# SRainGit/CAE-LO

Hardware: AMD Instinct MI355X
Metric: KITTI frames/sec end-to-end (keypts+desc+match+RANSAC) (higher is better)
Workload: dtype f32

## Files before the change

cae-lo_amd/csrc/encoder.hip:

```cpp
#include <math.h>

#include "caelo_internal.h"
#include <vector>
#include <stdlib.h>
#include <string.h>

typedef float f32x4 __attribute__((ext_vector_type(4)));

#define MFMA16(a, b, c) __builtin_amdgcn_mfma_f32_16x16x4f32((a), (b), (c), 0, 0, 0)

__device__ inline float enc_tanh(float x) {
    const float e = __builtin_amdgcn_exp2f(x * 2.8853900817779268f);
    return 1.0f - 2.0f * __builtin_amdgcn_rcpf(e + 1.0f);
}

#define DENSE_N 200
#define DENSE_NP 208
#define DENSE_K 2048
#define C3X_NPAIR 14
#define C3X_TICKET_INT 512
static void conv3_split_weights(const float *w3, uint4 *out);
static void stage1x_split_weights(const float *w1, const float *w2, uint4 *w1f, uint4 *w2x);
int enc_upload_dense1(const float *wd1, const float *bd1, int K, void **wx_dev, float **bd_dev);
#define HEAD_WQ_FLOATS (13 * 2 * 64 * 4)
// ... 247 lines not shown
                    const unsigned int n2 = (((w1 & 0xFFFFu) << 1) >> sh) & 0xFu, n3 = (((w1 >> 16) << 1) >> sh) & 0xFu;
                    m32[a >> 1] |= (n0 | (n1 << 4) | (n2 << 8) | (n3 << 12)) << ((a & 1) * 16);
                }
                cmask[rep] = (unsigned long long)m32[0] | ((unsigned long long)m32[1] << 32);
            }
        }
        int j_fetch;
        if (tid == 0) j_fetch = atomicAdd(work_counter, 1);
        ENC_STAMP(1);
#pragma unroll
        for (int rep = 0; rep < 2; ++rep) {
            const int cell = tid + rep * 256;
            const bool hit = cmask[rep] != 0ull;
            const unsigned long long bal = __ballot(hit);
            if (bal != 0ull) {
                int base = 0;
                if (lane == 0) base = atomicAdd(&L.list_n, __popcll(bal));
                base = __shfl(base, 0);
                if (hit) {
                    L.list_cell[base + __popcll(bal & ((1ull << lane) - 1ull))] = (unsigned short)cell;
                    L.cell_mask[cell] = cmask[rep];
                    atomicOr(&L.nzrow[(cell >> 6) + 1], 1u << (((cell >> 3) & 7) + 1));
                }
            }
        }
        caelo_lds_barrier();
        ENC_STAMP(2);
        const int nlist = L.list_n;
        for (int base = wave * 8; base < nlist; base += 32) {
            const int item = base + (lane >> 3);
            const int sub = lane & 7;
            float acc[8];
            int cell = 0;
            if (item < nlist) {
                cell = L.list_cell[item];
                const unsigned long long mask = L.cell_mask[cell];
                const int sa = sub >> 2, sb = (sub >> 1) & 1, sc = sub & 1;
                unsigned int taps = 0;
#pragma unroll
                for (int ka = 0; ka < 3; ++ka)
#pragma unroll
                    for (int kb = 0; kb < 3; ++kb)
                        taps |= ((unsigned int)(mask >> ((sa + ka) * 16 + (sb + kb) * 4 + sc)) & 7u) << ((ka * 3 + kb) * 3);
#pragma unroll
                for (int c = 0; c < 8; ++c) acc[c] = L.b1[c];
                while (taps) {
                    const int t = __ffs((int)taps) - 1;
                    taps &= taps - 1;
                    const float4 wa = *(const float4 *)&L.w1[t * 8], wb = *(const float4 *)&L.w1[t * 8 + 4];
                    acc[0] += wa.x; acc[1] += wa.y; acc[2] += wa.z; acc[3] += wa.w;
                    acc[4] += wb.x; acc[5] += wb.y; acc[6] += wb.z; acc[7] += wb.w;
                }
            } else {
#pragma unroll
                for (int c = 0; c < 8; ++c) acc[c] = -3.0e38f;
            }
#pragma unroll
            for (int c = 0; c < 8; ++c) {
                acc[c] = fmaxf(acc[c], __int_as_float(__builtin_amdgcn_update_dpp(0, __float_as_int(acc[c]), 0xB1, 0xF, 0xF, true)));
                acc[c] = fmaxf(acc[c], __int_as_float(__builtin_amdgcn_update_dpp(0, __float_as_int(acc[c]), 0x4E, 0xF, 0xF, true)));
                acc[c] = fmaxf(acc[c], __int_as_float(__builtin_amdgcn_update_dpp(0, __float_as_int(acc[c]), 0x141, 0xF, 0xF, true)));
            }
            if (item < nlist) {
                float mine = acc[0];
#pragma unroll
                for (int c = 1; c < 8; ++c) mine = (sub == c) ? acc[c] : mine;
                const int px = cell >> 6, py = (cell >> 3) & 7, pz = cell & 7;
                const int q = ((px + 1) * 10 + (py + 1)) * 10 + pz + 1;
                L.p1[(sub >> 2) * S1P_PLANE + q * 4 + (sub & 3)] = enc_tanh(mine) - L.bg[sub];
            }
        }
        if (tid == 0) L.next_j = (int)gridDim.x + j_fetch;
        caelo_lds_barrier();
        ENC_STAMP(3);
        const int jn = __builtin_amdgcn_readfirstlane(L.next_j);
        unsigned int row_next = 0u;
        if (jn < n_items) {
            const unsigned long long *src;
            enc_item(in, jn, nk, group, src, patch_next);
            patch_next = __builtin_amdgcn_readfirstlane(patch_next);
            row_next = ((const unsigned short *)src)[tid];
        }
        {
            const int yl = n >> 3, z = n & 7;
            const float *plane = L.p1 + (g >> 1) * S1P_PLANE + 2 * (g & 1);
#pragma unroll
            for (int yi = 0; yi < 4; ++yi) {
                const int y0 = 2 * yi;
                const int xp = wave ^ S1_XDEAL(yi);
                const unsigned int r0 = (unsigned)__builtin_amdgcn_readfirstlane((int)((L.nzrow[2 * xp] >> y0) & 0xFu));
                const unsigned int r1 = (unsigned)__builtin_amdgcn_readfirstlane((int)((L.nzrow[2 * xp + 1] >> y0) & 0xFu));
                const unsigned int r2 = (unsigned)__builtin_amdgcn_readfirstlane((int)((L.nzrow[2 * xp + 2] >> y0) & 0xFu));
                const unsigned int r3 = (unsigned)__builtin_amdgcn_readfirstlane((int)((L.nzrow[2 * xp + 3] >> y0) & 0xFu));
                float *dst = p2out + (size_t)patch * 1024 + (size_t)(((xp * 4 + yi) * 4 + 2 * (g & 1)) * 16 + n);
                if ((r0 | r1 | r2 | r3) == 0u) {
                    if (g < 2) {
                        const float2 o = L.bgout[wave][yi][lane];
                        dst[0] = o.x; dst[16] = o.y;
                    }
                    continue;
                }
                f32x4 acc0 = c0r[yi][0];
                f32x4 acc1 = c0r[yi][1];
                f32x4 acc0b = {0.f, 0.f, 0.f, 0.f}, acc1b = {0.f, 0.f, 0.f, 0.f};
                const int qbase = ((2 * xp) * 10 + (y0 + yl)) * 10 + z + 1;
                const float *a0 = plane + qbase * 4;
                const float *a1 = a0 + 100 * 4;
                CONV2Z_TILE(acc0, acc0b, a0, r0, r1, r2)
                CONV2Z_TILE(acc1, acc1b, a1, r1, r2, r3)
                acc0 += acc0b;
                acc1 += acc1b;
                float v0 = fmaxf(fmaxf(acc0[0], acc0[1]), fmaxf(acc1[0], acc1[1]));
                float v1 = fmaxf(fmaxf(acc0[2], acc0[3]), fmaxf(acc1[2], acc1[3]));
                v0 = fmaxf(v0, __shfl_xor(v0, 32));
                v1 = fmaxf(v1, __shfl_xor(v1, 32));
                if (g < 2) {
                    dst[0] = enc_tanh(v0);
                    dst[16] = enc_tanh(v1);
                }
            }
        }
        caelo_lds_barrier();
        ENC_STAMP(4);
#ifdef CAELO_ENC_PROF
        if (threadIdx.x == 0) { L.prof[6] += 1; L.prof[7] += nlist; }
#else
        if (threadIdx.x == 0 && blockIdx.x == 0 && patch == 0) g_enc_stamp[8] = (unsigned long long)nlist;
#endif
        for (int i = tid; i < nlist * 2; i += 256) {
            const int cell = L.list_cell[i >> 1];
            const int px = cell >> 6, py = (cell >> 3) & 7, pz = cell & 7;
            const int q = ((px + 1) * 10 + (py + 1)) * 10 + pz + 1;
            *(float4 *)&L.p1[(i & 1) * S1P_PLANE + q * 4] = make_float4(0.f, 0.f, 0.f, 0.f);
        }
        if (tid == 0) L.list_n = 0;
        if (tid < 12) L.nzrow[tid] = 0u;
        L.rows[rbuf ^ 1][row_slot] = (unsigned short)row_next;
        rbuf ^= 1;
        caelo_lds_barrier();
        j = jn;
        row = row_next;
        patch = patch_next;
        ENC_STAMP(5);
    }
#ifdef CAELO_ENC_PROF
    if (threadIdx.x == 0)
        for (int i = 0; i < 8; ++i) atomicAdd(&g_enc_stamp[i], (unsigned long long)L.prof[i]);
#endif
}

#include "enc_stage1x.inc"

#define ENC_XCD_CSTRIDE 32
#define C3X_PLANE 48
#define C3X_ARR 292
#define C3X_SPLIT (2 * C3X_ARR)
#ifndef C3X_F16
#define C3X_F16 1
#endif
#define C3X_NS (C3X_F16 ? 2 : 3)
#define C3X_SLOT (C3X_NS * C3X_SPLIT)
typedef __bf16 bf16x8 __attribute__((ext_vector_type(8)));
__host__ __device__ constexpr int c3x_pairA(int p) { return p < 9 ? p * 3 : (p < 12 ? (p - 9) * 9 + 2 : (p == 12 ? 8 : 26)); }
__host__ __device__ constexpr int c3x_pairB(int p) { return p < 9 ? p * 3 + 1 : (p < 12 ? (p - 9) * 9 + 5 : (p == 12 ? 17 : -1)); }
__host__ __device__ constexpr int c3x_pairClass(int p) { return p < 9 ? 0 : (p < 12 ? 1 : (p == 12 ? 2 : 3)); }
__host__ __device__ constexpr int c3x_tapPos(int t) { return (t / 9) * C3X_PLANE + ((t / 3) % 3) * 8 + (t % 3); }
__host__ __device__ constexpr bool c3x_dead(int x, int p) {
    return (x == 0 && c3x_pairA(p) / 9 == 0 && (c3x_pairB(p) < 0 || c3x_pairB(p) / 9 == 0)) ||
           (x == 3 && c3x_pairA(p) / 9 == 2 && (c3x_pairB(p) < 0 || c3x_pairB(p) / 9 == 2));
}

__host__ __device__ inline uint32_t enc_bf16_rne(float x) {
    union { float f; uint32_t u; } v = {x};
    return (v.u + 0x7FFFu + ((v.u >> 16) & 1u)) & 0xFFFF0000u;
}
__host__ __device__ inline float enc_bits_f32(uint32_t u) {
    union { uint32_t u; float f; } v = {u};
    return v.f;
}
__host__ __device__ inline void enc_split3(float x, uint32_t &hi, uint32_t &mid, uint32_t &lo) {
    hi = enc_bf16_rne(x);
    const float r = x - enc_bits_f32(hi);
    mid = enc_bf16_rne(r);
    lo = enc_bf16_rne(r - enc_bits_f32(mid));
}
__device__ inline void enc_split3_pk(float x0, float x1, uint32_t &hi, uint32_t &mid, uint32_t &lo) {
    typedef __bf16 enc_bf2 __attribute__((ext_vector_type(2)));
    typedef float enc_f2 __attribute__((ext_vector_type(2)));
    hi = __builtin_bit_cast(uint32_t, __builtin_convertvector((enc_f2){x0, x1}, enc_bf2));
    const float r0 = x0 - __uint_as_float(hi << 16), r1 = x1 - __uint_as_float(hi & 0xFFFF0000u);
    mid = __builtin_bit_cast(uint32_t, __builtin_convertvector((enc_f2){r0, r1}, enc_bf2));
    const float q0 = r0 - __uint_as_float(mid << 16), q1 = r1 - __uint_as_float(mid & 0xFFFF0000u);
    lo = __builtin_bit_cast(uint32_t, __builtin_convertvector((enc_f2){q0, q1}, enc_bf2));
}
__device__ inline void enc_split2h_pk(float x0, float x1, uint32_t &hi, uint32_t &lo) {
    const _Float16 h0 = (_Float16)x0, h1 = (_Float16)x1;
    const _Float16 l0 = (_Float16)(x0 - (float)h0), l1 = (_Float16)(x1 - (float)h1);
    hi = (uint32_t)__builtin_bit_cast(uint16_t, h0) | ((uint32_t)__builtin_bit_cast(uint16_t, h1) << 16);
    lo = (uint32_t)__builtin_bit_cast(uint16_t, l0) | ((uint32_t)__builtin_bit_cast(uint16_t, l1) << 16);
}
#define ENC_PK8(A) make_uint4((A[0] >> 16) | A[1], (A[2] >> 16) | A[3], (A[4] >> 16) | A[5], (A[6] >> 16) | A[7])

static void conv3_split_weights(const float *w3, uint4 *out) {
    for (int nt = 0; nt < 2; ++nt)
        for (int p = 0; p < C3X_NPAIR; ++p)
            for (int lane = 0; lane < 64; ++lane) {
                const int n = lane & 15, g = lane >> 4;
                const int tap = g < 2 ? c3x_pairA(p) : c3x_pairB(p);
                uint4 *o = out + ((size_t)(nt * C3X_NPAIR + p) * C3X_NS) * 64 + lane;
#if C3X_F16
                uint16_t h[8], l[8];
                for (int i = 0; i < 8; ++i)
                    enc_split2h(tap >= 0 ? w3[(tap * 16 + 8 * (g & 1) + i) * 32 + nt * 16 + n] : 0.0f, h[i], l[i]);
                o[0] = make_uint4(h[0] | (uint32_t)h[1] << 16, h[2] | (uint32_t)h[3] << 16, h[4] | (uint32_t)h[5] << 16, h[6] | (uint32_t)h[7] << 16);
                o[64] = make_uint4(l[0] | (uint32_t)l[1] << 16, l[2] | (uint32_t)l[3] << 16, l[4] | (uint32_t)l[5] << 16, l[6] | (uint32_t)l[7] << 16);
#else
                uint32_t h[8], m[8], l[8];
                for (int i = 0; i < 8; ++i)
                    enc_split3(tap >= 0 ? w3[(tap * 16 + 8 * (g & 1) + i) * 32 + nt * 16 + n] : 0.0f, h[i], m[i], l[i]);
                o[0] = ENC_PK8(h);
                o[64] = ENC_PK8(m);
                o[128] = ENC_PK8(l);
#endif
            }
}

#ifndef C3X_WGS
#define C3X_WGS 2
#endif
__global__ void __launch_bounds__(256, C3X_WGS) k_enc_conv3(const float *__restrict__ p2, int64_t n_patches, const caelo_enc_in in,
                                                      const uint4 *__restrict__ w3x, const float *__restrict__ b3g,
                                                      float *__restrict__ f3, int *__restrict__ stage1_counter,
                                                      int *__restrict__ xcd_counters) {
    __shared__ uint4 S[2 * C3X_SLOT];
    if (blockIdx.x == 0 && threadIdx.x == 0) *stage1_counter = 0;
    if (blockIdx.x == 0 && threadIdx.x < 8) xcd_counters[threadIdx.x * ENC_XCD_CSTRIDE] = 0;
    const int tid = threadIdx.x;
    const int lane = tid & 63;
    const int wave = tid >> 6;
    const int g = lane >> 4, n = lane & 15;
    const int ntile = wave & 1, slot = __builtin_amdgcn_readfirstlane(wave >> 1);
    uint4 bq[C3X_NPAIR][C3X_NS];
#pragma unroll
    for (int p = 0; p < C3X_NPAIR; ++p)
#pragma unroll
        for (int sp = 0; sp < C3X_NS; ++sp) bq[p][sp] = w3x[((size_t)(ntile * C3X_NPAIR + p) * C3X_NS + sp) * 64 + lane];
    const float bias = b3g[16 * ntile + n];
    for (int i = tid; i < 2 * C3X_SLOT; i += 256) S[i] = make_uint4(0u, 0u, 0u, 0u);
    __syncthreads();
    const int n_items = enc_items_total(in, n_patches);
    const int n_pairs = (n_items + 1) / 2;
#define C3_ROW(ITEM, ROW)                                     \
    {                                                         \
        ROW = (ITEM);                                         \
        if (in.dedup) {                                       \
            int f_, i_;                                       \
            ROW = enc_item_row(in, (ITEM), f_, i_);           \
        }                                                     \
    }
    const int f_slot = __builtin_amdgcn_readfirstlane(tid >> 7), f_pos = (tid >> 1) & 63, f_h = tid & 1;
    const int f_q = (((f_pos >> 4) + 1) * 6 + ((f_pos >> 2) & 3) + 1) * 8 + (f_pos & 3) + 1;
    float4 pre0, pre1;
#define C3_FETCH(PAIR)                                                                           \
    {                                                                                            \
        const int pa_ = (PAIR) * 2 + f_slot;                                                     \
        pre0 = make_float4(0.f, 0.f, 0.f, 0.f);                                                  \
        pre1 = pre0;                                                                             \
        if ((PAIR) < n_pairs && pa_ < n_items) {                                                 \
            int row_;                                                                            \
            C3_ROW(pa_, row_)                                                                    \
            const float4 *q_ = (const float4 *)(p2 + (size_t)row_ * 1024 + f_pos * 16 + 8 * f_h); \
            pre0 = q_[0];                                                                        \
            pre1 = q_[1];                                                                        \
        }                                                                                        \
    }
#ifdef CAELO_C3_PROF
    unsigned long long c3_t[4] = {0ull, 0ull, 0ull, 0ull};
    unsigned c3_prev = (unsigned)clock64();
#define C3_STAMP(i) do { if (tid == 0) { const unsigned t_ = (unsigned)clock64(); c3_t[i] += t_ - c3_prev; c3_prev = t_; } } while (0)
#else
#define C3_STAMP(i) do { } while (0)
#endif
    __shared__ int s_after[2];
    const int xcd = (int)(blockIdx.x & 7u), wgs_of_xcd = ((int)gridDim.x - xcd + 7) >> 3;
    int *const ticket = stage1_counter + C3X_TICKET_INT + 32 * xcd;
    int pair = xcd + 8 * (int)(blockIdx.x >> 3), next = pair + 8 * wgs_of_xcd;
    int drawn = 0;
    if (tid == 0) drawn = atomicAdd(ticket, 1);
    C3_FETCH(pair)
    for (int it = 0; pair < n_pairs; pair = next, next = __builtin_amdgcn_readfirstlane(s_after[it & 1]), ++it) {
        C3_STAMP(3);
        {
            const float v[8] = {pre0.x, pre0.y, pre0.z, pre0.w, pre1.x, pre1.y, pre1.z, pre1.w};
            uint4 *d = &S[f_slot * C3X_SLOT + f_h * C3X_ARR + f_q];
#if C3X_F16
            uint32_t h[4], l[4];
#pragma unroll
            for (int k = 0; k < 4; ++k) enc_split2h_pk(v[2 * k], v[2 * k + 1], h[k], l[k]);
            d[0] = make_uint4(h[0], h[1], h[2], h[3]);
            d[C3X_SPLIT] = make_uint4(l[0], l[1], l[2], l[3]);
#else
            uint32_t h[4], m[4], l[4];
#pragma unroll
            for (int k = 0; k < 4; ++k) enc_split3_pk(v[2 * k], v[2 * k + 1], h[k], m[k], l[k]);
            d[0] = make_uint4(h[0], h[1], h[2], h[3]);
            d[C3X_SPLIT] = make_uint4(m[0], m[1], m[2], m[3]);
            d[2 * C3X_SPLIT] = make_uint4(l[0], l[1], l[2], l[3]);
#endif
        }
        if (tid == 0) s_after[it & 1] = xcd + 8 * (2 * wgs_of_xcd + drawn);
        C3_STAMP(0);
        __syncthreads();
        C3_STAMP(1);
        if (tid == 0) drawn = atomicAdd(ticket, 1);
        C3_FETCH(next)
        const int item = pair * 2 + slot;
        int patch;
        C3_ROW(item, patch)
        const uint4 *base = &S[slot * C3X_SLOT + (g & 1) * C3X_ARR + (n >> 2) * 8 + (n & 3)];
        const uint4 *ab[4] = {base + (g >= 2 ? 1 : 0), base + (g >= 2 ? 8 : 0), base + (g >= 2 ? C3X_PLANE : 0), base};
#pragma unroll
        for (int round = 0; round < 2; ++round) {
            f32x4 acc[2];
#pragma unroll
            for (int j = 0; j < 2; ++j) acc[j] = (f32x4){bias, bias, bias, bias};
#pragma unroll
            for (int p = 0; p < C3X_NPAIR; ++p) {
#if C3X_F16
                typedef _Float16 c3_h8 __attribute__((ext_vector_type(8)));
                const c3_h8 bh = __builtin_bit_cast(c3_h8, bq[p][0]), bl = __builtin_bit_cast(c3_h8, bq[p][1]);
                c3_h8 ah[2], al[2];
#pragma unroll
                for (int j = 0; j < 2; ++j) {
                    if (c3x_dead(2 * round + j, p)) continue;
                    const uint4 *a = ab[c3x_pairClass(p)] + c3x_tapPos(c3x_pairA(p)) + (2 * round + j) * C3X_PLANE;
                    ah[j] = __builtin_bit_cast(c3_h8, a[0]);
                    al[j] = __builtin_bit_cast(c3_h8, a[C3X_SPLIT]);
                }
#define C3X_MAC(A, B)                                                                                           \
    _Pragma("unroll") for (int j = 0; j < 2; ++j) if (!c3x_dead(2 * round + j, p))                              \
        acc[j] = __builtin_amdgcn_mfma_f32_16x16x32_f16(A[j], B, acc[j], 0, 0, 0);
                C3X_MAC(al, bh)
                C3X_MAC(ah, bl)
                C3X_MAC(ah, bh)
#else
                const bf16x8 bh = __builtin_bit_cast(bf16x8, bq[p][0]), bm = __builtin_bit_cast(bf16x8, bq[p][1]),
                             bl = __builtin_bit_cast(bf16x8, bq[p][2]);
                bf16x8 ah[2], am[2], al[2];
#pragma unroll
                for (int j = 0; j < 2; ++j) {
                    if (c3x_dead(2 * round + j, p)) continue;
                    const uint4 *a = ab[c3x_pairClass(p)] + c3x_tapPos(c3x_pairA(p)) + (2 * round + j) * C3X_PLANE;
                    ah[j] = __builtin_bit_cast(bf16x8, a[0]);
                    am[j] = __builtin_bit_cast(bf16x8, a[C3X_SPLIT]);
                    al[j] = __builtin_bit_cast(bf16x8, a[2 * C3X_SPLIT]);
                }
#define C3X_MAC(A, B)                                                                                           \
    _Pragma("unroll") for (int j = 0; j < 2; ++j) if (!c3x_dead(2 * round + j, p))                              \
        acc[j] = __builtin_amdgcn_mfma_f32_16x16x32_bf16(A[j], B, acc[j], 0, 0, 0);
                C3X_MAC(al, bh)
                C3X_MAC(ah, bl)
                C3X_MAC(am, bm)
                C3X_MAC(am, bh)
                C3X_MAC(ah, bm)
                C3X_MAC(ah, bh)
#endif
            }
            if (item < n_items) {
                float *dst = f3 + (size_t)patch * 2048 + 16 * ntile + n;
#pragma unroll
                for (int j = 0; j < 2; ++j)
#pragma unroll
                    for (int r = 0; r < 4; ++r) dst[(((2 * round + j) * 4 + g) * 4 + r) * 32] = enc_tanh(acc[j][r]);
            }
        }
        C3_STAMP(2);
        __syncthreads();
    }
#ifdef CAELO_C3_PROF
    if (tid == 0) {
        for (int i = 0; i < 4; ++i) atomicAdd(&g_enc_stamp[8 + i], c3_t[i]);
        atomicAdd(&g_enc_stamp[12], 1ull);
    }
#endif
}

#define D1_BM 64
#define D1_BK 32
#define D1_SPLIT 8
#ifndef D1_SPLIT_2048
#define D1_SPLIT_2048 2
#endif
#define D1_SPLIT_OF(KTOT) ((KTOT) > 2048 ? 8 : D1_SPLIT_2048)
#define D1_THREADS 512
#define D1_NT (DENSE_NP / 16)
#define D1_NS 2
#define D1_B16 (D1_NS * D1_NT * 64)
#define D1_BSLOTS ((D1_B16 + D1_THREADS - 1) / D1_THREADS)

static void dense1_split_weights(const float *wd1, int K, uint4 *out) {
    for (int ks = 0; ks < K / 32; ++ks)
        for (int nt = 0; nt < D1_NT; ++nt)
            for (int lane = 0; lane < 64; ++lane) {
                const int n = lane & 15, g = lane >> 4, col = nt * 16 + n;
                uint16_t h[8], l[8];
                for (int i = 0; i < 8; ++i)
                    enc_split2h(col < DENSE_N ? wd1[(size_t)(ks * 32 + 8 * g + i) * DENSE_N + col] : 0.0f, h[i], l[i]);
                uint4 *o = out + (size_t)ks * D1_B16 + nt * 64 + lane;
                o[0] = make_uint4(h[0] | (uint32_t)h[1] << 16, h[2] | (uint32_t)h[3] << 16, h[4] | (uint32_t)h[5] << 16, h[6] | (uint32_t)h[7] << 16);
                o[D1_NT * 64] = make_uint4(l[0] | (uint32_t)l[1] << 16, l[2] | (uint32_t)l[3] << 16, l[4] | (uint32_t)l[5] << 16, l[6] | (uint32_t)l[7] << 16);
            }
}

int enc_upload_dense1(const float *wd1, const float *bd1, int K, void **wx_dev, float **bd_dev) {
    const size_t n = (size_t)(K / 32) * D1_B16;
    uint4 *wx = (uint4 *)malloc(n * sizeof(uint4));
    if (!wx) { caelo_set_error("out of host memory"); return CAELO_ERR_ARG; }
    dense1_split_weights(wd1, K, wx);
    float bd[DENSE_NP] = {0.0f};
    memcpy(bd, bd1, DENSE_N * sizeof(float));
    hipError_t e = hipSuccess;
    if (!*wx_dev) e = hipMalloc(wx_dev, (n + 6 * 64) * sizeof(uint4));
    if (e == hipSuccess && !*bd_dev) e = hipMalloc((void **)bd_dev, sizeof(bd));
    if (e == hipSuccess) e = hipMemcpy(*wx_dev, wx, n * sizeof(uint4), hipMemcpyHostToDevice);
    if (e == hipSuccess) e = hipMemcpy(*bd_dev, bd, sizeof(bd), hipMemcpyHostToDevice);
    free(wx);
    if (e != hipSuccess) { caelo_set_error("dense_1 upload failed: %s", hipGetErrorString(e)); return CAELO_ERR_HIP; }
    return CAELO_OK;
}

typedef _Float16 d1_h8 __attribute__((ext_vector_type(8)));
#define D1_MFMA(A, B, C) __builtin_amdgcn_mfma_f32_16x16x32_f16((A), (B), (C), 0, 0, 0)

#define D1P_BSTRIDE (26 * 64)
#define D1P_NBUF(MTW) 3
#define D1P_LDS_BYTES(MTW) ((2 * D1_NS * 4 * D1_BM * (MTW) + D1P_NBUF(MTW) * D1P_BSTRIDE) * 16)
template <int KTOT, int MTW>
__global__ void __launch_bounds__(D1_THREADS, 2) k_enc_dense1p(const float *__restrict__ f3, int64_t n_rows_pad,
                                                               const uint4 *__restrict__ wd1x, float *__restrict__ part,
                                                               const caelo_enc_in in) {
    constexpr int BM = D1_BM * MTW, A16 = D1_NS * 4 * BM, NBUF = D1P_NBUF(MTW), NKS = KTOT / D1_SPLIT_OF(KTOT) / D1_BK;
    constexpr int DMA = 4;
    constexpr int PER_STAGE = DMA + MTW;
    static_assert(MTW >= 1 && MTW <= 3, "three instances");
    static_assert(NKS % 2 == 0 && NKS >= 6, "stages are unrolled in pairs, the last ones peeled");
    int64_t row0 = (int64_t)blockIdx.x * BM;
    int split = blockIdx.y;
    if (in.dedup) {
        const int lin = (int)(blockIdx.y * gridDim.x + blockIdx.x);
        int t = lin / D1_SPLIT_OF(KTOT), f = 0;
        split = lin - t * D1_SPLIT_OF(KTOT);
        for (; f < in.n_frames; ++f) {
            const int live = (enc_tables(in, f)->count + BM - 1) / BM;
            if (t < live) break;
            t -= live;
        }
        if (f == in.n_frames) return;
        row0 = (int64_t)f * in.per_frame + (int64_t)t * BM;
    }
    extern __shared__ uint4 d1_lds[];
    uint4 *As = d1_lds;
    uint4 *Bs = d1_lds + 2 * A16;
    const int tid = threadIdx.x;
    const int lane = tid & 63, wave = __builtin_amdgcn_readfirstlane(tid >> 6);
    const int g = lane >> 4, n = lane & 15;
    const int ks0 = split * NKS;
    const int mg = wave >> 1;
    const bool odd = (wave & 1) != 0;
    const int nt0 = odd ? 7 : 0;
    f32x4 acc[MTW][7];
#pragma unroll
    for (int q = 0; q < MTW; ++q)
#pragma unroll
        for (int i = 0; i < 7; ++i) acc[q][i] = (f32x4){0.f, 0.f, 0.f, 0.f};
    const int a_row = wave * 8 + ((lane >> 1) & 7), a_kq = ((lane >> 4) << 1) | (lane & 1);
    const float *a_src = f3 + (size_t)(row0 + a_row) * KTOT + (size_t)ks0 * D1_BK + a_kq * 4;
    const int pb = wave < 6 ? 4 * wave : 22;
    const uint32_t b_lds = (uint32_t)(uintptr_t)(void __attribute__((address_space(3))) *)(Bs + (pb + 1) * 64);
    const uint4 *b_mid = wd1x + (size_t)ks0 * D1_B16 + (pb + 1) * 64 + lane;
    const uint32_t a_lds = (uint32_t)(uintptr_t)(void __attribute__((address_space(3))) *)&As[(a_kq >> 1) * BM + a_row] + (a_kq & 1) * 8;
    f32x4 paA[MTW], paB[MTW];
    d1_h8 af0[MTW][D1_NS], af1[MTW][D1_NS], bf0[4][D1_NS], bf1[3][D1_NS];
#define D1P_FETCH_B(KS, BUF)                                                                                     \
    {                                                                                                            \
        const uint4 *gp_ = b_mid + (size_t)(KS) * D1_B16;                                                        \
        const uint32_t la_ = b_lds + (uint32_t)(BUF) * (D1P_BSTRIDE * 16u);                                      \
        __asm__ volatile("s_mov_b32 m0, %0\n\ts_nop 0\n\t"                                                       \
                         "global_load_lds_dwordx4 %1, off offset:-1024\n\t"                                       \
                         "global_load_lds_dwordx4 %1, off\n\tglobal_load_lds_dwordx4 %1, off offset:1024\n\t"    \
                         "global_load_lds_dwordx4 %1, off offset:2048" : : "s"(la_), "v"(gp_) : "memory");       \
    }
#define D1P_LOAD_A(P, KS)                                                                                        \
    _Pragma("unroll") for (int r = 0; r < MTW; ++r) {                                                            \
        const float *p_ = a_src + (size_t)(64 * r) * KTOT + (size_t)(KS) * D1_BK;                                \
        __asm__ volatile("global_load_dwordx4 %0, %1, off" : "=v"(P[r]) : "v"(p_) : "memory");                   \
    }
#define D1P_WAIT_A(P, N)                                                                                         \
    {                                                                                                            \
        if (MTW == 1) __asm__ volatile("s_waitcnt vmcnt(%1)" : "+v"(P[0]) : "n"(N) : "memory");                  \
        else __asm__ volatile("s_waitcnt vmcnt(%2)" : "+v"(P[0]), "+v"(P[MTW - 1]) : "n"(N) : "memory");         \
    }
#define D1P_STORE_A(P, ABUF)                                                                               \
    _Pragma("unroll") for (int r = 0; r < MTW; ++r) {                                                      \
        uint32_t h01_, l01_, h23_, l23_;                                                                   \
        enc_split2h_pk(P[r][0], P[r][1], h01_, l01_);                                                      \
        enc_split2h_pk(P[r][2], P[r][3], h23_, l23_);                                                      \
        const unsigned long long dh_ = ((unsigned long long)h23_ << 32) | h01_, dl_ = ((unsigned long long)l23_ << 32) | l01_; \
        if (r == 0)                                                                                        \
            __asm__ volatile("ds_write_b64 %0, %1 offset:%3\n\tds_write_b64 %0, %2 offset:%4"               \
                             : : "v"(a_lds), "v"(dh_), "v"(dl_), "n"((ABUF) * A16 * 16),                     \
                                 "n"((ABUF) * A16 * 16 + 4 * BM * 16) : "memory");                          \
        else if (r == 1)                                                                                   \
            __asm__ volatile("ds_write_b64 %0, %1 offset:%3\n\tds_write_b64 %0, %2 offset:%4"               \
                             : : "v"(a_lds), "v"(dh_), "v"(dl_), "n"((ABUF) * A16 * 16 + 1024),              \
                                 "n"((ABUF) * A16 * 16 + 4 * BM * 16 + 1024) : "memory");                   \
        else                                                                                               \
            __asm__ volatile("ds_write_b64 %0, %1 offset:%3\n\tds_write_b64 %0, %2 offset:%4"               \
                             : : "v"(a_lds), "v"(dh_), "v"(dl_), "n"((ABUF) * A16 * 16 + 2048),              \
                                 "n"((ABUF) * A16 * 16 + 4 * BM * 16 + 2048) : "memory");                   \
    }
#define D1P_READ_A(AF, ABUF)                                                                               \
    _Pragma("unroll") for (int q = 0; q < MTW; ++q) {                                                      \
        const uint4 *ap_ = &As[(ABUF) * A16 + g * BM + (mg * MTW + q) * 16 + n];                           \
        AF[q][0] = __builtin_bit_cast(d1_h8, ap_[0]);                                                      \
        AF[q][1] = __builtin_bit_cast(d1_h8, ap_[4 * BM]);                                                 \
    }
#define D1P_READ_B0(BUF)                                                                                   \
    {                                                                                                      \
// ... 158 lines not shown
        int r_ = enc_tables(in, (int)f_)->slot_of[p - f_ * per_in];
        if (r_ < 0) {
            const unsigned g_ = (unsigned)(-r_ - 1), fr_ = g_ / per_in;
            r_ = enc_tables(in, (int)fr_)->slot_of[g_ - fr_ * per_in];
        }
        row = (unsigned)r_;
    }
    const float *src = part + (size_t)row * DENSE_NP + 4 * g;
    float4 v[HM_JW][SPLIT];
#pragma unroll
    for (int c = 0; c < HM_JW; ++c)
#pragma unroll
        for (int sp = 0; sp < SPLIT; ++sp)
            if (wave + 4 * c < D1_NT) v[c][sp] = *(const float4 *)(src + (size_t)sp * n_rows_pad * DENSE_NP + 16 * (wave + 4 * c));
    f32x4 acc0 = {0.f, 0.f, 0.f, 0.f}, acc1 = {0.f, 0.f, 0.f, 0.f};
#pragma unroll
    for (int c = 0; c < HM_JW; ++c) {
        if (wave + 4 * c < D1_NT) {
            float4 sum = b1[c];
#pragma unroll
            for (int sp = 0; sp < SPLIT; ++sp) { sum.x += v[c][sp].x; sum.y += v[c][sp].y; sum.z += v[c][sp].z; sum.w += v[c][sp].w; }
            const float hv[4] = {enc_tanh(sum.x), enc_tanh(sum.y), enc_tanh(sum.z), enc_tanh(sum.w)};
            const float w0[4] = {wq[c][0].x, wq[c][0].y, wq[c][0].z, wq[c][0].w}, w1[4] = {wq[c][1].x, wq[c][1].y, wq[c][1].z, wq[c][1].w};
#pragma unroll
            for (int i = 0; i < 4; ++i) {
                acc0 = __builtin_amdgcn_mfma_f32_16x16x4f32(hv[i], w0[i], acc0, 0, 0, 0);
                acc1 = __builtin_amdgcn_mfma_f32_16x16x4f32(hv[i], w1[i], acc1, 0, 0, 0);
            }
        }
    }
    if (wave > 0) {
        s_c[wave - 1][0][lane] = acc0;
        s_c[wave - 1][1][lane] = acc1;
    }
    __syncthreads();
    if (wave > 0) return;
#pragma unroll
    for (int w = 0; w < 3; ++w) {
        acc0 += s_c[w][0][lane];
        acc1 += s_c[w][1][lane];
    }
    const float bo0 = bd2[m], bo1 = m < 4 ? bd2[16 + m] : 0.0f;
#pragma unroll
    for (int i = 0; i < 4; ++i) {
        const unsigned pp = tile * 16u + 4u * (unsigned)g + (unsigned)i;
        if (pp < n_all) {
            const unsigned f = pp / per_out, q = pp - f * per_out, kp = q / (unsigned)group;
            float *dst = outs.base[f] + (size_t)kp * out_stride + (size_t)(q - kp * (unsigned)group) * 20;
            const float d0 = enc_tanh(bo0 + acc0[i]);
            dst[m] = d0;
            if (!(fabsf(d0) <= 1.0f)) atomicAdd(faults, 1);
            if (m < 4) {
                const float d1 = enc_tanh(bo1 + acc1[i]);
                dst[16 + m] = d1;
                if (!(fabsf(d1) <= 1.0f)) atomicAdd(faults, 1);
            }
        }
    }
}

static inline int64_t pad64(int64_t n) { return (n + D1_BM - 1) / D1_BM * D1_BM; }


CAELO_API int64_t caelo_encode_ws_bytes(int64_t n_patches) {
    const int64_t np = pad64(n_patches);
    return CAELO_ENC_WS_HEADER + (np * 1024 + np * 2048 + (int64_t)D1_SPLIT * np * DENSE_NP) * (int64_t)sizeof(float);
}

CAELO_API int caelo_encode_ws_layout(int64_t n_patches, int64_t out[6]) {
    CAELO_REQUIRE(out && n_patches > 0, "caelo_encode_ws_layout: bad argument");
    const int64_t np = pad64(n_patches);
    out[0] = CAELO_ENC_WS_HEADER;
    out[1] = out[0] + np * 1024 * (int64_t)sizeof(float);
    out[2] = out[1] + np * 2048 * (int64_t)sizeof(float);
    out[3] = np;
    out[4] = D1_SPLIT_OF(DENSE_K);
    out[5] = D1_SPLIT;
    return CAELO_OK;
}

int encode_impl(caelo_ctx *c, const uint64_t *bits, int64_t n_patches, int group, float *out, int out_stride,
                       void *ws, hipStream_t s, hipEvent_t *ev ) {
    CAELO_REQUIRE(out, "null argument");
    caelo_enc_out outs;
    outs.base[0] = out;
    outs.per_frame = n_patches > 0 ? n_patches : 1;
    return encode_batch_impl(c, bits, n_patches, group, outs, out_stride, ws, s, ev);
}

int encode_batch_impl(caelo_ctx *c, const uint64_t *bits, int64_t n_patches, int group, const caelo_enc_out &outs,
                      int out_stride, void *ws, hipStream_t s, hipEvent_t *ev , const caelo_enc_in *in) {
    CAELO_REQUIRE(c && bits && ws, "null argument");
    const caelo_enc_in ein = in ? *in : caelo_enc_in{(const unsigned long long *)bits, 0, (int32_t)(n_patches < 0x7FFFFFFF ? n_patches : 0), 1, 0, 0};
    CAELO_REQUIRE(!ein.dedup || (ein.n_frames >= 1 && ein.n_frames <= CAELO_ENC_MAX_FRAMES && ein.per_frame % (3 * D1_BM) == 0 &&
                                 (int64_t)ein.n_frames * ein.per_frame == n_patches),
                  "bad de-duplicated launch");
    CAELO_REQUIRE(outs.per_frame > 0 && (n_patches + outs.per_frame - 1) / outs.per_frame <= CAELO_ENC_MAX_FRAMES, "bad frame table");
    CAELO_REQUIRE(!ein.dedup || ein.per_frame == CAELO_FRAME_PATCHES, "de-duplicated launches hold whole frames of 3072 patches");
    CAELO_REQUIRE(c->has_enc, "encoder weights not set (caelo_set_encoder_weights)");
    CAELO_REQUIRE(n_patches > 0 && n_patches < 0x7FFFFFFF && group >= 1 && out_stride >= group * 20, "bad shape");
    const int64_t np = pad64(n_patches);
    int *work_counter = (int *)ws;
    unsigned long long *mfma_count = (unsigned long long *)((char *)ws + CAELO_ENC_WS_MFMA);
    float *p2 = (float *)((char *)ws + CAELO_ENC_WS_HEADER);
    float *f3 = p2 + np * 1024;
    float *part = f3 + np * 2048;
    if (np > n_patches)
        CAELO_HIP(hipMemsetAsync(f3 + n_patches * 2048, 0, (size_t)(np - n_patches) * 2048 * sizeof(float), s));
    const bool stage1x = !c->enc_reference;
    static int slots1x_slot[CAELO_MAX_DEVICES];
    static bool slots1x_have[CAELO_MAX_DEVICES];
    static std::mutex slots1x_mu;
    const int slots1x = per_device_once(c->device, slots1x_slot, slots1x_have, slots1x_mu, [&] {
        int per_cu = 0, cus = 0;
        if (hipOccupancyMaxActiveBlocksPerMultiprocessor(&per_cu, (const void *)k_enc_stage1x<false>, 256, 0) != hipSuccess ||
            hipDeviceGetAttribute(&cus, hipDeviceAttributeMultiprocessorCount, c->device) != hipSuccess || per_cu * cus <= 0)
            return 512;
        return per_cu * cus;
    });
    int *xcd_counters = (int *)((char *)ws + 1024);
    static int slots1_slot[CAELO_MAX_DEVICES];
    static bool slots1_have[CAELO_MAX_DEVICES];
    static std::mutex slots1_mu;
    const int slots1 = per_device_once(c->device, slots1_slot, slots1_have, slots1_mu, [&] {
        int per_cu = 0, cus = 0;
        if (hipOccupancyMaxActiveBlocksPerMultiprocessor(&per_cu, (const void *)k_enc_stage1, 256, 0) != hipSuccess ||
            hipDeviceGetAttribute(&cus, hipDeviceAttributeMultiprocessorCount, c->device) != hipSuccess || per_cu * cus <= 0)
            return 768;
        return per_cu * cus;
    });
    const int64_t cap1 = (ein.yield & 1) ? (int64_t)slots1 * 4 / 5 : slots1;
    const unsigned g1 = (unsigned)(n_patches < cap1 ? n_patches : cap1);
    if (ev) CAELO_HIP(hipEventRecord(ev[0], s));
    const int order_group = (n_patches % group == 0) ? group : 1;
    if (stage1x) {
        static const int slots_env = getenv("CAELO_S1X_SLOTS") ? atoi(getenv("CAELO_S1X_SLOTS")) : 0;
        const int64_t capx = slots_env > 0 ? slots_env : ((ein.yield & 1) ? (int64_t)slots1x * 2 / 3 : slots1x);
        const unsigned gx = (unsigned)(n_patches < capx ? n_patches : capx);
        if (ev) {
            CAELO_HIP(hipMemsetAsync(mfma_count, 0, 1024, s));
            CAELO_HIP(hipEventRecord(ev[0], s));
            k_enc_stage1x<true><<<gx, 256, 0, s>>>(ein, n_patches, order_group, work_counter, (const uint4 *)c->enc_w1f, c->enc_b1,
                                                   (const uint4 *)c->enc_w2x, c->enc_c0, p2, mfma_count);
        } else
            k_enc_stage1x<false><<<gx, 256, 0, s>>>(ein, n_patches, order_group, work_counter, (const uint4 *)c->enc_w1f, c->enc_b1,
                                                    (const uint4 *)c->enc_w2x, c->enc_c0, p2, mfma_count);
        CAELO_LAUNCH_CHECK();
    } else {
        if (ev) CAELO_HIP(hipMemsetAsync(mfma_count, 0, 1024, s));
        k_enc_stage1<<<g1, 256, 0, s>>>(ein, n_patches, order_group, work_counter, c->enc_w1, c->enc_b1, c->enc_w2, c->enc_c0, p2);
        CAELO_LAUNCH_CHECK();
    }
    if (ev) CAELO_HIP(hipEventRecord(ev[1], s));
    const int64_t pairs = (n_patches + 1) / 2;
    const int64_t cap3 = ((ein.yield & 2) ? 256 : ((ein.yield & 4) ? 384 : 512)) * C3X_WGS / 2;
    const unsigned g3 = (unsigned)(pairs < cap3 ? pairs : cap3);
    k_enc_conv3<<<g3, 256, 0, s>>>(p2, n_patches, ein, (const uint4 *)c->enc_w3x, c->enc_b3, f3, work_counter, xcd_counters);
    CAELO_LAUNCH_CHECK();
    if (ev) CAELO_HIP(hipEventRecord(ev[2], s));
    {
        const int rc = dense1_launch<DENSE_K>(c->device, f3, np, c->enc_wd1x, part, ein, s);
        if (rc) return rc;
    }
    if (ev) CAELO_HIP(hipEventRecord(ev[3], s));
    k_enc_head_mfma<D1_SPLIT_OF(DENSE_K)><<<(unsigned)((n_patches + 15) / 16), 256, 0, s>>>(part, n_patches, np, c->enc_bd1, (const float4 *)c->enc_wd2q,
                                                                                       c->enc_bd2, group, outs, out_stride, ein, c->faults);
    CAELO_LAUNCH_CHECK();
    if (ev) CAELO_HIP(hipEventRecord(ev[4], s));
    return CAELO_OK;
}

int64_t enc_dense_pad(int64_t n) { return pad64(n); }
int64_t enc_dense32_part_bytes(int64_t np) { return (int64_t)D1_SPLIT * np * DENSE_NP * (int64_t)sizeof(float); }
int enc_dense32_head_launch(caelo_ctx *c, const float *f3, int64_t n_patches, int64_t np, float *part, int group, float *out,
                            int out_stride, hipStream_t s) {
    const caelo_enc_in plain = {nullptr, 0, (int32_t)n_patches, 1, 0, 0};
    {
        const int rc = dense1_launch<16384>(c->device, f3, np, c->enc32_wd1x, part, plain, s);
        if (rc) return rc;
    }
    caelo_enc_out outs = {};
    outs.base[0] = out;
    outs.per_frame = n_patches;
    k_enc_head_mfma<D1_SPLIT_OF(16384)><<<(unsigned)((n_patches + 15) / 16), 256, 0, s>>>(part, n_patches, np, c->enc32_bd1, (const float4 *)c->enc_wd2q,
                                                                                     c->enc_bd2, group, outs, out_stride, plain, c->faults);
    CAELO_LAUNCH_CHECK();
    return CAELO_OK;
}

CAELO_API int caelo_encode(caelo_ctx *c, const uint64_t *bits, int64_t n_patches, int group, float *out,
                           int out_stride, void *ws, void *stream) {
    return encode_impl(c, bits, n_patches, group, out, out_stride, ws, caelo_stream(stream), nullptr);
}

CAELO_API int caelo_encode_profile(caelo_ctx *c, const uint64_t *bits, int64_t n_patches, int group, float *out,
                                   int out_stride, void *ws, void *stream, float *ms_host) {
    CAELO_REQUIRE(ms_host != nullptr, "null argument");
    hipStream_t s = caelo_stream(stream);
    hipEvent_t ev[5];
    for (int i = 0; i < 5; ++i) CAELO_HIP(hipEventCreate(&ev[i]));
    int rc = encode_impl(c, bits, n_patches, group, out, out_stride, ws, s, ev);
    if (rc == CAELO_OK) {
        CAELO_HIP(hipEventSynchronize(ev[4]));
        for (int i = 0; i < 4; ++i) CAELO_HIP(hipEventElapsedTime(&ms_host[i], ev[i], ev[i + 1]));
        unsigned long long rows = 0, part[128];
        CAELO_HIP(hipMemcpy(part, (char *)ws + CAELO_ENC_WS_MFMA, sizeof(part), hipMemcpyDeviceToHost));
        for (int i = 0; i < 8; ++i) rows += part[16 * i];
        const bool f32_kernel = c->enc_reference;
        ms_host[4] = (float)((double)rows * (f32_kernel ? 6.0 : 1.0) / 1e6);
        ms_host[5] = f32_kernel ? 2.0f * 16 * 16 * 4 : 2.0f * 16 * 16 * 32;
    }
    for (int i = 0; i < 5; ++i) (void)hipEventDestroy(ev[i]);
    return rc;
}

CAELO_API int caelo_set_encoder_reference(caelo_ctx *c, int on) {
    CAELO_REQUIRE(c, "null argument");
    c->enc_reference = on != 0;
    return CAELO_OK;
}
```

Measured before the change: 18780.

## Retile conv3 MFMA so M dimension spans 16 patches per output position

Rewrites the conv3 encoder kernel so that each MFMA's 16-row M dimension covers 16 different patches at one spatial position, not 16 positions of a single patch. Work items become (16-patch tile, x-plane) units that stage three input x-planes in LDS, with compile-time tap offsets and dead-tap skipping generated by templates. Boundary taps read a shared zero slab. The dedup row lookup becomes a prefix table in LDS, and the next prefetch now sits between the two output rows. The aim is fewer wasted MFMAs on padded positions and better weight reuse, at the cost of more prefetch registers (12 float4), larger LDS staging, and dropping the bf16 3-way path.

```diff
diff --git a/cae-lo_amd/csrc/encoder.hip b/cae-lo_amd/csrc/encoder.hip
--- a/cae-lo_amd/csrc/encoder.hip
+++ b/cae-lo_amd/csrc/encoder.hip
@@ -423,23 +423,42 @@
 #include "enc_stage1x.inc"
 
 #define ENC_XCD_CSTRIDE 32
-#define C3X_PLANE 48
-#define C3X_ARR 292
-#define C3X_SPLIT (2 * C3X_ARR)
 #ifndef C3X_F16
 #define C3X_F16 1
 #endif
+#if !C3X_F16
+#error "k_enc_conv3 implements the f16 x 2 split only (the 3-way bf16 form is conv3_split_weights' alone)"
+#endif
 #define C3X_NS (C3X_F16 ? 2 : 3)
-#define C3X_SLOT (C3X_NS * C3X_SPLIT)
-typedef __bf16 bf16x8 __attribute__((ext_vector_type(8)));
+#define C3T_POS 64
+#define C3T_PLANE (16 * C3T_POS)
+#define C3T_ZERO (3 * C3T_PLANE)
+#define C3T_LDS (C3T_ZERO + C3T_POS)
 __host__ __device__ constexpr int c3x_pairA(int p) { return p < 9 ? p * 3 : (p < 12 ? (p - 9) * 9 + 2 : (p == 12 ? 8 : 26)); }
 __host__ __device__ constexpr int c3x_pairB(int p) { return p < 9 ? p * 3 + 1 : (p < 12 ? (p - 9) * 9 + 5 : (p == 12 ? 17 : -1)); }
-__host__ __device__ constexpr int c3x_pairClass(int p) { return p < 9 ? 0 : (p < 12 ? 1 : (p == 12 ? 2 : 3)); }
-__host__ __device__ constexpr int c3x_tapPos(int t) { return (t / 9) * C3X_PLANE + ((t / 3) % 3) * 8 + (t % 3); }
-__host__ __device__ constexpr bool c3x_dead(int x, int p) {
-    return (x == 0 && c3x_pairA(p) / 9 == 0 && (c3x_pairB(p) < 0 || c3x_pairB(p) / 9 == 0)) ||
-           (x == 3 && c3x_pairA(p) / 9 == 2 && (c3x_pairB(p) < 0 || c3x_pairB(p) / 9 == 2));
-}
+__host__ __device__ constexpr int c3t_tap(int t, int xc, int y, int z) {
+    return ((xc == 0 && t / 9 == 0) || (xc == 2 && t / 9 == 2) || y + (t / 3) % 3 - 1 < 0 || y + (t / 3) % 3 - 1 > 3 ||
+            z + t % 3 - 1 < 0 || z + t % 3 - 1 > 3)
+               ? -1
+               : (t / 9) * C3T_PLANE + ((y + (t / 3) % 3 - 1) * 4 + z + t % 3 - 1) * C3T_POS;
+}
+__host__ __device__ constexpr bool c3t_live(int p, int xc, int y, int z) {
+    return c3t_tap(c3x_pairA(p), xc, y, z) >= 0 || (c3x_pairB(p) >= 0 && c3t_tap(c3x_pairB(p), xc, y, z) >= 0);
+}
+__host__ __device__ constexpr int c3t_off(int p, int h, int xc, int y, int z) {
+    return c3t_tap(h && c3x_pairB(p) >= 0 ? c3x_pairB(p) : c3x_pairA(p), xc, y, z) < 0
+               ? C3T_ZERO
+               : c3t_tap(h && c3x_pairB(p) >= 0 ? c3x_pairB(p) : c3x_pairA(p), xc, y, z);
+}
+__host__ __device__ constexpr int c3t_live_slabs() {
+    int s = 0;
+    for (int x = 0; x < 4; ++x)
+        for (int y = 0; y < 4; ++y)
+            for (int z = 0; z < 4; ++z)
+                for (int p = 0; p < C3X_NPAIR; ++p) s += c3t_live(p, x == 0 ? 0 : (x == 3 ? 2 : 1), y, z) ? 1 : 0;
+    return s;
+}
+static_assert(c3t_live_slabs() == 583, "583 / 16 = 36.4 slabs per patch and n-tile");
 
 __host__ __device__ inline uint32_t enc_bf16_rne(float x) {
     union { float f; uint32_t u; } v = {x};
@@ -499,51 +518,109 @@
 #ifndef C3X_WGS
 #define C3X_WGS 2
 #endif
+__device__ inline int c3t_tile(int w) { return (w >> 5) * 8 + (w & 7); }
+__device__ inline int c3t_xplane(int w) { return (w >> 3) & 3; }
+__host__ __device__ inline int64_t c3t_works(int64_t n_items) { return 32 * ((n_items + 127) / 128); }
+typedef _Float16 c3_h8 __attribute__((ext_vector_type(8)));
+
+template <int XC, int Y, int P>
+__device__ __forceinline__ void c3t_pair(const uint4 *__restrict__ S, int loff, int upm, const uint4 (&bq)[C3X_NPAIR][C3X_NS],
+                                         f32x4 (&acc)[4]) {
+    constexpr bool live[4] = {c3t_live(P, XC, Y, 0), c3t_live(P, XC, Y, 1), c3t_live(P, XC, Y, 2), c3t_live(P, XC, Y, 3)};
+    constexpr int oa[4] = {c3t_off(P, 0, XC, Y, 0), c3t_off(P, 0, XC, Y, 1), c3t_off(P, 0, XC, Y, 2), c3t_off(P, 0, XC, Y, 3)};
+    constexpr int ob[4] = {c3t_off(P, 1, XC, Y, 0), c3t_off(P, 1, XC, Y, 1), c3t_off(P, 1, XC, Y, 2), c3t_off(P, 1, XC, Y, 3)};
+    if (!(live[0] || live[1] || live[2] || live[3])) return;
+    const c3_h8 bh = __builtin_bit_cast(c3_h8, bq[P][0]), bl = __builtin_bit_cast(c3_h8, bq[P][1]);
+    c3_h8 ah[4], al[4];
+#pragma unroll
+    for (int z = 0; z < 4; ++z) {
+        if (!live[z]) continue;
+        const uint4 *a = S + (loff + (upm & (ob[z] - oa[z]))) + oa[z];
+        ah[z] = __builtin_bit_cast(c3_h8, a[0]);
+        al[z] = __builtin_bit_cast(c3_h8, a[32]);
+    }
+#define C3T_MAC(A, B)                                                                                       \
+    _Pragma("unroll") for (int z = 0; z < 4; ++z) if (live[z])                                             \
+        acc[z] = __builtin_amdgcn_mfma_f32_16x16x32_f16(A[z], B, acc[z], 0, 0, 0);
+    C3T_MAC(al, bh)
+    C3T_MAC(ah, bl)
+    C3T_MAC(ah, bh)
+#undef C3T_MAC
+}
+template <int XC, int Y, int P>
+struct C3tPairs {
+    static __device__ __forceinline__ void run(const uint4 *__restrict__ S, int loff, int upm, const uint4 (&bq)[C3X_NPAIR][C3X_NS],
+                                               f32x4 (&acc)[4]) {
+        c3t_pair<XC, Y, P>(S, loff, upm, bq, acc);
+        C3tPairs<XC, Y, P + 1>::run(S, loff, upm, bq, acc);
+    }
+};
+template <int XC, int Y>
+struct C3tPairs<XC, Y, C3X_NPAIR> {
+    static __device__ __forceinline__ void run(const uint4 *__restrict__, int, int, const uint4 (&)[C3X_NPAIR][C3X_NS], f32x4 (&)[4]) {}
+};
+template <int XC, int Y>
+__device__ __forceinline__ void c3t_row(const uint4 *__restrict__ S, int loff, int upm, const uint4 (&bq)[C3X_NPAIR][C3X_NS],
+                                        float bias, f32x4 (&acc)[4]) {
+#pragma unroll
+    for (int z = 0; z < 4; ++z) acc[z] = (f32x4){bias, bias, bias, bias};
+    C3tPairs<XC, Y, 0>::run(S, loff, upm, bq, acc);
+}
+
 __global__ void __launch_bounds__(256, C3X_WGS) k_enc_conv3(const float *__restrict__ p2, int64_t n_patches, const caelo_enc_in in,
                                                       const uint4 *__restrict__ w3x, const float *__restrict__ b3g,
                                                       float *__restrict__ f3, int *__restrict__ stage1_counter,
                                                       int *__restrict__ xcd_counters) {
-    __shared__ uint4 S[2 * C3X_SLOT];
+    __shared__ uint4 S[C3T_LDS];
+    __shared__ int4 s_rows[4];
     if (blockIdx.x == 0 && threadIdx.x == 0) *stage1_counter = 0;
     if (blockIdx.x == 0 && threadIdx.x < 8) xcd_counters[threadIdx.x * ENC_XCD_CSTRIDE] = 0;
     const int tid = threadIdx.x;
     const int lane = tid & 63;
     const int wave = tid >> 6;
     const int g = lane >> 4, n = lane & 15;
-    const int ntile = wave & 1, slot = __builtin_amdgcn_readfirstlane(wave >> 1);
+    const int ntile = wave & 1, yh = __builtin_amdgcn_readfirstlane(wave >> 1);
     uint4 bq[C3X_NPAIR][C3X_NS];
 #pragma unroll
     for (int p = 0; p < C3X_NPAIR; ++p)
 #pragma unroll
         for (int sp = 0; sp < C3X_NS; ++sp) bq[p][sp] = w3x[((size_t)(ntile * C3X_NPAIR + p) * C3X_NS + sp) * 64 + lane];
     const float bias = b3g[16 * ntile + n];
-    for (int i = tid; i < 2 * C3X_SLOT; i += 256) S[i] = make_uint4(0u, 0u, 0u, 0u);
+    __shared__ int s_first[CAELO_ENC_MAX_FRAMES];
+    if (tid < C3T_POS) S[C3T_ZERO + tid] = make_uint4(0u, 0u, 0u, 0u);
+    if (tid == 0 && in.dedup)
+        for (int f = 0, acc = 0; f < in.n_frames; ++f) {
+            s_first[f] = acc;
+            acc += enc_tables(in, f)->count;
+        }
+    const int n_items = enc_items_total(in, n_patches);
     __syncthreads();
-    const int n_items = enc_items_total(in, n_patches);
-    const int n_pairs = (n_items + 1) / 2;
-#define C3_ROW(ITEM, ROW)                                     \
-    {                                                         \
-        ROW = (ITEM);                                         \
-        if (in.dedup) {                                       \
-            int f_, i_;                                       \
-            ROW = enc_item_row(in, (ITEM), f_, i_);           \
-        }                                                     \
-    }
-    const int f_slot = __builtin_amdgcn_readfirstlane(tid >> 7), f_pos = (tid >> 1) & 63, f_h = tid & 1;
-    const int f_q = (((f_pos >> 4) + 1) * 6 + ((f_pos >> 2) & 3) + 1) * 8 + (f_pos & 3) + 1;
-    float4 pre0, pre1;
-#define C3_FETCH(PAIR)                                                                           \
-    {                                                                                            \
-        const int pa_ = (PAIR) * 2 + f_slot;                                                     \
-        pre0 = make_float4(0.f, 0.f, 0.f, 0.f);                                                  \
-        pre1 = pre0;                                                                             \
-        if ((PAIR) < n_pairs && pa_ < n_items) {                                                 \
-            int row_;                                                                            \
-            C3_ROW(pa_, row_)                                                                    \
-            const float4 *q_ = (const float4 *)(p2 + (size_t)row_ * 1024 + f_pos * 16 + 8 * f_h); \
-            pre0 = q_[0];                                                                        \
-            pre1 = q_[1];                                                                        \
-        }                                                                                        \
+    const int n_work = (int)c3t_works(n_items);
+    const int f_item = tid & 15, f_h = (tid >> 4) & 1, f_pos = (tid >> 5) & 7;
+    float4 pre[12];
+    int f_row;
+#define C3T_FETCH(W)                                                                                      \
+    {                                                                                                     \
+        const int it_ = c3t_tile(W) * 16 + f_item, x_ = c3t_xplane(W);                                    \
+        f_row = -1;                                                                                       \
+        _Pragma("unroll") for (int k = 0; k < 12; ++k) pre[k] = make_float4(0.f, 0.f, 0.f, 0.f);          \
+        if ((W) < n_work && it_ < n_items) {                                                              \
+            f_row = it_;                                                                                  \
+            if (in.dedup) {    \
+                int f_ = 0;                                                                               \
+                for (int k_ = 1; k_ < in.n_frames; ++k_) f_ += s_first[k_] <= it_ ? 1 : 0;               \
+                f_row = f_ * in.per_frame + it_ - s_first[f_];                                            \
+            }                                                                                             \
+            const float *q_ = p2 + (size_t)f_row * 1024 + f_pos * 16 + 8 * f_h;                           \
+            _Pragma("unroll") for (int k = 0; k < 6; ++k) {                                               \
+                const int xin_ = x_ - 1 + (k >> 1);                                                       \
+                if (xin_ >= 0 && xin_ < 4) {                                                              \
+                    const float4 *v_ = (const float4 *)(q_ + xin_ * 256 + (k & 1) * 128);                 \
+                    pre[2 * k] = v_[0];                                                                   \
+                    pre[2 * k + 1] = v_[1];                                                               \
+                }                                                                                         \
+            }                                                                                             \
+        }                                                                                                 \
     }
 #ifdef CAELO_C3_PROF
     unsigned long long c3_t[4] = {0ull, 0ull, 0ull, 0ull};
@@ -555,96 +632,54 @@
     __shared__ int s_after[2];
     const int xcd = (int)(blockIdx.x & 7u), wgs_of_xcd = ((int)gridDim.x - xcd + 7) >> 3;
     int *const ticket = stage1_counter + C3X_TICKET_INT + 32 * xcd;
-    int pair = xcd + 8 * (int)(blockIdx.x >> 3), next = pair + 8 * wgs_of_xcd;
+    int w = xcd + 8 * (int)(blockIdx.x >> 3), next = w + 8 * wgs_of_xcd;
     int drawn = 0;
     if (tid == 0) drawn = atomicAdd(ticket, 1);
-    C3_FETCH(pair)
-    for (int it = 0; pair < n_pairs; pair = next, next = __builtin_amdgcn_readfirstlane(s_after[it & 1]), ++it) {
+    C3T_FETCH(w)
+    for (int it = 0; w < n_work; w = next, next = __builtin_amdgcn_readfirstlane(s_after[it & 1]), ++it) {
         C3_STAMP(3);
-        {
-            const float v[8] = {pre0.x, pre0.y, pre0.z, pre0.w, pre1.x, pre1.y, pre1.z, pre1.w};
-            uint4 *d = &S[f_slot * C3X_SLOT + f_h * C3X_ARR + f_q];
-#if C3X_F16
+#pragma unroll
+        for (int k = 0; k < 6; ++k) {
+            const float v[8] = {pre[2 * k].x, pre[2 * k].y, pre[2 * k].z, pre[2 * k].w,
+                                pre[2 * k + 1].x, pre[2 * k + 1].y, pre[2 * k + 1].z, pre[2 * k + 1].w};
             uint32_t h[4], l[4];
 #pragma unroll
-            for (int k = 0; k < 4; ++k) enc_split2h_pk(v[2 * k], v[2 * k + 1], h[k], l[k]);
+            for (int kk = 0; kk < 4; ++kk) enc_split2h_pk(v[2 * kk], v[2 * kk + 1], h[kk], l[kk]);
+            uint4 *d = &S[(k >> 1) * C3T_PLANE + (f_pos + 8 * (k & 1)) * C3T_POS + f_h * 16 + f_item];
             d[0] = make_uint4(h[0], h[1], h[2], h[3]);
-            d[C3X_SPLIT] = make_uint4(l[0], l[1], l[2], l[3]);
-#else
-            uint32_t h[4], m[4], l[4];
-#pragma unroll
-            for (int k = 0; k < 4; ++k) enc_split3_pk(v[2 * k], v[2 * k + 1], h[k], m[k], l[k]);
-            d[0] = make_uint4(h[0], h[1], h[2], h[3]);
-            d[C3X_SPLIT] = make_uint4(m[0], m[1], m[2], m[3]);
-            d[2 * C3X_SPLIT] = make_uint4(l[0], l[1], l[2], l[3]);
-#endif
-        }
+            d[32] = make_uint4(l[0], l[1], l[2], l[3]);
+        }
+        if (tid < 16) ((int *)s_rows)[tid] = f_row;
         if (tid == 0) s_after[it & 1] = xcd + 8 * (2 * wgs_of_xcd + drawn);
         C3_STAMP(0);
         __syncthreads();
         C3_STAMP(1);
         if (tid == 0) drawn = atomicAdd(ticket, 1);
-        C3_FETCH(next)
-        const int item = pair * 2 + slot;
-        int patch;
-        C3_ROW(item, patch)
-        const uint4 *base = &S[slot * C3X_SLOT + (g & 1) * C3X_ARR + (n >> 2) * 8 + (n & 3)];
-        const uint4 *ab[4] = {base + (g >= 2 ? 1 : 0), base + (g >= 2 ? 8 : 0), base + (g >= 2 ? C3X_PLANE : 0), base};
-#pragma unroll
-        for (int round = 0; round < 2; ++round) {
-            f32x4 acc[2];
-#pragma unroll
-            for (int j = 0; j < 2; ++j) acc[j] = (f32x4){bias, bias, bias, bias};
-#pragma unroll
-            for (int p = 0; p < C3X_NPAIR; ++p) {
-#if C3X_F16
-                typedef _Float16 c3_h8 __attribute__((ext_vector_type(8)));
-                const c3_h8 bh = __builtin_bit_cast(c3_h8, bq[p][0]), bl = __builtin_bit_cast(c3_h8, bq[p][1]);
-                c3_h8 ah[2], al[2];
-#pragma unroll
-                for (int j = 0; j < 2; ++j) {
-                    if (c3x_dead(2 * round + j, p)) continue;
-                    const uint4 *a = ab[c3x_pairClass(p)] + c3x_tapPos(c3x_pairA(p)) + (2 * round + j) * C3X_PLANE;
-                    ah[j] = __builtin_bit_cast(c3_h8, a[0]);
-                    al[j] = __builtin_bit_cast(c3_h8, a[C3X_SPLIT]);
-                }
-#define C3X_MAC(A, B)                                                                                           \
-    _Pragma("unroll") for (int j = 0; j < 2; ++j) if (!c3x_dead(2 * round + j, p))                              \
-        acc[j] = __builtin_amdgcn_mfma_f32_16x16x32_f16(A[j], B, acc[j], 0, 0, 0);
-                C3X_MAC(al, bh)
-                C3X_MAC(ah, bl)
-                C3X_MAC(ah, bh)
-#else
-                const bf16x8 bh = __builtin_bit_cast(bf16x8, bq[p][0]), bm = __builtin_bit_cast(bf16x8, bq[p][1]),
-                             bl = __builtin_bit_cast(bf16x8, bq[p][2]);
-                bf16x8 ah[2], am[2], al[2];
-#pragma unroll
-                for (int j = 0; j < 2; ++j) {
-                    if (c3x_dead(2 * round + j, p)) continue;
-                    const uint4 *a = ab[c3x_pairClass(p)] + c3x_tapPos(c3x_pairA(p)) + (2 * round + j) * C3X_PLANE;
-                    ah[j] = __builtin_bit_cast(bf16x8, a[0]);
-                    am[j] = __builtin_bit_cast(bf16x8, a[C3X_SPLIT]);
-                    al[j] = __builtin_bit_cast(bf16x8, a[2 * C3X_SPLIT]);
-                }
-#define C3X_MAC(A, B)                                                                                           \
-    _Pragma("unroll") for (int j = 0; j < 2; ++j) if (!c3x_dead(2 * round + j, p))                              \
-        acc[j] = __builtin_amdgcn_mfma_f32_16x16x32_bf16(A[j], B, acc[j], 0, 0, 0);
-                C3X_MAC(al, bh)
-                C3X_MAC(ah, bl)
-                C3X_MAC(am, bm)
-                C3X_MAC(am, bh)
-                C3X_MAC(ah, bm)
-                C3X_MAC(ah, bh)
-#endif
-            }
-            if (item < n_items) {
-                float *dst = f3 + (size_t)patch * 2048 + 16 * ntile + n;
-#pragma unroll
-                for (int j = 0; j < 2; ++j)
-#pragma unroll
-                    for (int r = 0; r < 4; ++r) dst[(((2 * round + j) * 4 + g) * 4 + r) * 32] = enc_tanh(acc[j][r]);
-            }
-        }
+        const int tile = c3t_tile(w), X = c3t_xplane(w);
+        const bool live = tile * 16 < n_items;
+        const int xc = X == 0 ? 0 : (X == 3 ? 2 : 1);
+        const int4 rows = s_rows[g];
+        int loff = (g & 1) * 16 + n, upm = g >= 2 ? -1 : 0;
+        asm volatile("" : "+v"(loff), "+v"(upm));
+        f32x4 acc[4];
+#define C3T_CASE(XC, YH, YY) case (XC) * 2 + (YH): c3t_row<XC, 2 * (YH) + (YY)>(S, loff, upm, bq, bias, acc); break;
+#define C3T_ROW(YY)                                                                                          \
+        switch (xc * 2 + yh) {                                                                               \
+            C3T_CASE(0, 0, YY) C3T_CASE(0, 1, YY) C3T_CASE(1, 0, YY) C3T_CASE(1, 1, YY) C3T_CASE(2, 0, YY)   \
+            default: C3T_CASE(2, 1, YY)                                                                      \
+        }                                                                                                    \
+        {                                            \
+            const int rr[4] = {rows.x, rows.y, rows.z, rows.w};                                              \
+            _Pragma("unroll") for (int r = 0; r < 4; ++r) if (rr[r] >= 0) {                                  \
+                float *dst = f3 + (size_t)rr[r] * 2048 + (X * 4 + 2 * yh + (YY)) * 128 + 16 * ntile + n;     \
+                _Pragma("unroll") for (int z = 0; z < 4; ++z) dst[z * 32] = enc_tanh(acc[z][r]);             \
+            }                                                                                                \
+        }
+        if (live) { C3T_ROW(0) }
+        C3T_FETCH(next)
+        if (live) { C3T_ROW(1) }
+#undef C3T_ROW
+#undef C3T_CASE
         C3_STAMP(2);
         __syncthreads();
     }
@@ -1109,9 +1144,9 @@
         CAELO_LAUNCH_CHECK();
     }
     if (ev) CAELO_HIP(hipEventRecord(ev[1], s));
-    const int64_t pairs = (n_patches + 1) / 2;
+    const int64_t works = c3t_works(n_patches);
     const int64_t cap3 = ((ein.yield & 2) ? 256 : ((ein.yield & 4) ? 384 : 512)) * C3X_WGS / 2;
-    const unsigned g3 = (unsigned)(pairs < cap3 ? pairs : cap3);
+    const unsigned g3 = (unsigned)(works < cap3 ? works : cap3);
     k_enc_conv3<<<g3, 256, 0, s>>>(p2, n_patches, ein, (const uint4 *)c->enc_w3x, c->enc_b3, f3, work_counter, xcd_counters);
     CAELO_LAUNCH_CHECK();
     if (ev) CAELO_HIP(hipEventRecord(ev[2], s));
```

Result: faster. 19060 (median of 6 runs) (+1.4%).
